# ShifuML/shifu-tensorflow

Hardware: NVIDIA H100
Metric: rows/sec tabular-DNN train (higher is better)
Workload: dtype bf16

## Files before the change

shifu-tensorflow_b200/csrc/capi.cu:

```cuda
#include <math.h>
#include <stdlib.h>
#include <string.h>
#include <algorithm>
#include <memory>
#include <random>
#include "net.cuh"
#include "gemm_dw.cuh"
#include "gemm_pp.cuh"
#include "savedmodel.h"
#include "xchg_p2p.cuh"

using namespace sb;

enum { G_STEP = 0, G_ACC = 1, G_KINDS = 2 };

struct sb_trainer {
  Net net;
  sb_net_desc desc;
  OptHyper hyper;
  float lr = 0.f;
  int rank = 0, world = 1;
  NcclComm comm = nullptr;
  float *grad = nullptr, *s1 = nullptr, *s2 = nullptr, *acc = nullptr;
  int n_acc = 0;
  float grad_out_scale = 1.f;
  long long global_step = 0;
  float* h_scal = nullptr;
  float* d_hscal = nullptr;
  enum { HIST = 8192 };
  float2* h_hist = nullptr;
  float2* d_hist = nullptr;
  float2* hist_slot(long long step) { return d_hist ? d_hist + (step % HIST) : nullptr; }
  float *dsX = nullptr, *dsY = nullptr, *dsW = nullptr;
  __nv_bfloat16* dsXb = nullptr;
  int* dsP = nullptr;
  long long ds_rows = 0;
  std::map<std::pair<int, int>, cudaGraphExec_t> graphs;
  std::map<int, int> kernels_per_step;
  void* xch = nullptr;
  long long xch_n4 = 0;
  long long grad_off = 0, flags_off = 0;
  P2PFlags* flags = nullptr;
  P2PPeers* d_peers = nullptr;
  std::vector<void*> peer_bases;
  bool p2p_ready = false;
  bool peers_share_device = false;
  bool grad_sharded = false;
  bool master_stale = false;
  unsigned int epoch = 0;
  unsigned int* h_err = nullptr;
  unsigned int* d_herr = nullptr;
  unsigned long long xchg_timeout_ns = 300ull * 1000000000ull;
  int xchg_blocks = 0;
  int x_chunks = 1, x_slots = 2;
  int x_chunk_rows = 0;
  int x_begin[SB_XCHG_SLOTS] = {}, x_end[SB_XCHG_SLOTS] = {};
  cudaEvent_t ev_x[SB_XCHG_SLOTS] = {};
  cudaEvent_t ev_c[SB_XCHG_SLOTS] = {};
  bool ll_ready = false;
  long long llg_off = 0, lls_off = 0;
  cudaStream_t side = nullptr;
// ... 1431 lines not shown
  SB_CUDA(cudaMalloc(&dA32, sizeof(float) * M * K));
  SB_CUDA(cudaMalloc(&dB32, sizeof(float) * N * K));
  SB_CUDA(cudaMalloc(&dD, sizeof(float) * M * N));
  SB_CUDA(cudaMalloc(&dA, sizeof(__nv_bfloat16) * a_rows * lda));
  SB_CUDA(cudaMalloc(&dB, sizeof(__nv_bfloat16) * b_rows * ldb));
  SB_CUDA(cudaMemset(dA, 0, sizeof(__nv_bfloat16) * a_rows * lda));
  SB_CUDA(cudaMemset(dB, 0, sizeof(__nv_bfloat16) * b_rows * ldb));
  SB_CUDA(cudaMemset(dD, 0, sizeof(float) * M * N));
  SB_CUDA(cudaMemcpy(dA32, A, sizeof(float) * M * K, cudaMemcpyHostToDevice));
  SB_CUDA(cudaMemcpy(dB32, B, sizeof(float) * N * K, cudaMemcpyHostToDevice));
  cast_bf16_kernel<<<static_cast<unsigned>((static_cast<long long>(M) * K + 255) / 256), 256>>>(dA32, a_rows, a_cols, dA, lda);
  cast_bf16_kernel<<<static_cast<unsigned>((static_cast<long long>(N) * K + 255) / 256), 256>>>(dB32, b_rows, b_cols, dB, ldb);
  GemmPlan pl = plan_gemm(M, N, K, prop.multiProcessorCount, false);
  if (cfg_cg > 0) pl.bn = cfg_bn;
  {
    const int total_kb = (K + 63) / 64;
    int want = split_k < 1 ? 1 : (split_k > total_kb ? total_kb : split_k);
    pl.kb_per_split = (total_kb + want - 1) / want;
    pl.split_k = (total_kb + pl.kb_per_split - 1) / pl.kb_per_split;
    const int work = ((M + 127) / 128) * ((N + pl.bn - 1) / pl.bn) * pl.split_k;
    pl.grid = work < prop.multiProcessorCount ? work : prop.multiProcessorCount;
  }
  TmapSet tms;
  int s = make_tmap_bf16(&tms.a[0], dA, a_rows, a_cols, lda, a_mn ? 64 : 128);
  if (s == SB_OK) s = make_tmap_bf16(&tms.b[0], dB, b_rows, b_cols, ldb, b_mn ? 64 : pl.bn);
  if (s == SB_OK) {
    GemmTcParams p = {};
    p.M = M; p.N = N; p.K = K;
    p.accum = dD; p.ld_acc = N;
    p.acc_vec4 = (N % 4 == 0) ? 1 : 0;
    auto launch = [&]() -> int {
      if (pl.bn == 256) return launch_gemm_dw(pl, tms, p, 0);
      if (!a_mn && !b_mn) return launch_gemm_tc<EPI_F32, false, false>(pl, tms, p, 0);
      if (!a_mn) return launch_gemm_tc<EPI_F32, false, true>(pl, tms, p, 0);
      return launch_gemm_tc<EPI_F32, true, true>(pl, tms, p, 0);
    };
    if (pl.bn == 256) s = set_gemm_dw_attrs();
    else if (!a_mn && !b_mn) s = set_gemm_tc_attrs<EPI_F32, false, false>();
    else if (!a_mn) s = set_gemm_tc_attrs<EPI_F32, false, true>();
    else s = set_gemm_tc_attrs<EPI_F32, true, true>();
    if (s == SB_OK) s = launch();
    if (s == SB_OK && iters > 0) {
      const int ldn = round_up(N, 8);
      float *d_bias = nullptr, *d_colsum = nullptr;
      __nv_bfloat16 *d_out = nullptr, *d_aux = nullptr;
      cudaMalloc(&d_bias, sizeof(float) * N); cudaMemset(d_bias, 0, sizeof(float) * N);
      cudaMalloc(&d_colsum, sizeof(float) * N); cudaMemset(d_colsum, 0, sizeof(float) * N);
      cudaMalloc(&d_out, sizeof(__nv_bfloat16) * static_cast<size_t>(M) * ldn);
      cudaMalloc(&d_aux, sizeof(__nv_bfloat16) * static_cast<size_t>(M) * ldn);
      cudaMemset(d_aux, 0x3f, sizeof(__nv_bfloat16) * static_cast<size_t>(M) * ldn);
      GemmTcParams q = p;
      q.bias = d_bias; q.act = SB_ACT_RELU; q.out = d_out; q.ld_out = ldn; q.aux = d_aux; q.ld_aux = ldn; q.colsum = d_colsum;
      q.acc_vec4 = (N % 4 == 0) ? 1 : 0;
      const PpPlan pp = plan_gemm_pp(M, N, K, prop.multiProcessorCount);
      PpTmaps pt;
      if (!a_mn) {
        if (s == SB_OK) s = make_tmap_bf16(&pt.a, dA, a_rows, a_cols, lda, pp.bm_wg);
        if (s == SB_OK) s = make_tmap_bf16(&pt.b, dB, b_rows, b_cols, ldb, b_mn ? 64 : pp.bn);
        if (s == SB_OK) s = make_tmap_bf16(&pt.o, d_out, M, N, ldn, pp.bm_wg);
        if (s == SB_OK) s = make_tmap_bf16(&pt.x, d_aux, M, N, ldn, pp.bm_wg);
      }
      auto real = [&]() -> int {
        if (!a_mn && !b_mn) return launch_gemm_pp<EPI_DA>(pp, pt, q, 0, false);
        if (!a_mn) return launch_gemm_pp<EPI_FWD>(pp, pt, q, 0, false);
        if (pl.bn == 256) return launch_gemm_dw(pl, tms, q, 0, false);
        return launch_gemm_tc<EPI_DW, true, true>(pl, tms, q, 0, false);
      };
      if (s == SB_OK) s = a_mn ? set_gemm_tc_attrs<EPI_DW, true, true>() : set_gemm_pp_attrs();
      cudaEvent_t e0, e1;
      cudaEventCreate(&e0); cudaEventCreate(&e1);
      for (int i = 0; i < 3 && s == SB_OK; ++i) s = real();
      cudaEventRecord(e0, 0);
      for (int i = 0; i < iters && s == SB_OK; ++i) s = real();
      cudaEventRecord(e1, 0);
      cudaEventSynchronize(e1);
      float ms = 0.f;
      cudaEventElapsedTime(&ms, e0, e1);
      *ms_out = ms / iters;
      cudaEventDestroy(e0); cudaEventDestroy(e1);
      if (getenv("SB_GEMM_TRACE")) {
        unsigned long long* d_tr = nullptr;
        cudaMalloc(&d_tr, 16 * sizeof(unsigned long long));
        cudaMemset(d_tr, 0, 16 * sizeof(unsigned long long));
        q.trace = d_tr;
        cudaDeviceSynchronize();
        cudaEvent_t t0, t1;
        cudaEventCreate(&t0); cudaEventCreate(&t1);
        cudaEventRecord(t0, 0);
        s = real();
        cudaEventRecord(t1, 0);
        cudaEventSynchronize(t1);
        float one = 0.f;
        cudaEventElapsedTime(&one, t0, t1);
        unsigned long long h[16];
        cudaMemcpy(h, d_tr, sizeof(h), cudaMemcpyDeviceToHost);
        if (a_mn)
          fprintf(stderr, "[trace] M=%d N=%d K=%d bn=%d split=%d single-launch %.2f us | ns since entry:", M, N, K, pl.bn, pl.split_k,
                  one * 1e3f);
        else
          fprintf(stderr, "[trace] M=%d N=%d K=%d ping-pong bm_wg=%d bn=%d single-launch %.2f us | ns since entry:", M, N, K, pp.bm_wg,
                  pp.bn, one * 1e3f);
        const char* nm[9] = {"entry", "setup", "deps", "tma0", "land0", "mma_done", "acc_ready", "epi_done", "exit"};
        for (int i = 1; i < 9; ++i) fprintf(stderr, " %s=%lld", nm[i], (long long)(h[i] - h[0]));
        fprintf(stderr, "\n");
        cudaEventDestroy(t0); cudaEventDestroy(t1);
        cudaFree(d_tr);
        q.trace = nullptr;
      }
      cudaFree(d_bias); cudaFree(d_colsum); cudaFree(d_out); cudaFree(d_aux);
    }
  }
  if (s == SB_OK) {
    cudaError_t e = cudaDeviceSynchronize();
    if (e != cudaSuccess) s = set_error(SB_ERR_CUDA, "gemm_tc_kernel failed: %s", cudaGetErrorString(e));
    else if (cudaMemcpy(D, dD, sizeof(float) * M * N, cudaMemcpyDeviceToHost) != cudaSuccess) s = set_error(SB_ERR_CUDA, "D2H failed");
  }
  cudaFree(dA32); cudaFree(dB32); cudaFree(dD); cudaFree(dA); cudaFree(dB);
  return s;
}

extern "C" {
// ... 5 lines not shown
  cudaDeviceProp prop;
  SB_CUDA(cudaGetDeviceProperties(&prop, device));
  SB_CHECK(prop.major == 9 && prop.minor == 0, SB_ERR_CUDA, "device is sm_%d%d, need sm_90", prop.major, prop.minor);
  SB_CUDA(cudaSetDevice(device));
  const int ld = round_up(K, 8);
  const long long a_ps = static_cast<long long>(M) * ld, b_ps = static_cast<long long>(N) * ld;
  float *dA32 = nullptr, *dB32 = nullptr, *dD = nullptr;
  __nv_bfloat16 *dA = nullptr, *dB = nullptr;
  SB_CUDA(cudaMalloc(&dA32, sizeof(float) * M * K));
  SB_CUDA(cudaMalloc(&dB32, sizeof(float) * N * K));
  SB_CUDA(cudaMalloc(&dD, sizeof(float) * M * N));
  SB_CUDA(cudaMalloc(&dA, sizeof(__nv_bfloat16) * a_ps * np));
  SB_CUDA(cudaMalloc(&dB, sizeof(__nv_bfloat16) * b_ps * np));
  SB_CUDA(cudaMemset(dA, 0, sizeof(__nv_bfloat16) * a_ps * np));
  SB_CUDA(cudaMemset(dB, 0, sizeof(__nv_bfloat16) * b_ps * np));
  SB_CUDA(cudaMemset(dD, 0, sizeof(float) * M * N));
  SB_CUDA(cudaMemcpy(dA32, A, sizeof(float) * M * K, cudaMemcpyHostToDevice));
  SB_CUDA(cudaMemcpy(dB32, B, sizeof(float) * N * K, cudaMemcpyHostToDevice));
  cast_bf16_kernel<<<static_cast<unsigned>((static_cast<long long>(M) * K + 255) / 256), 256>>>(dA32, M, K, dA, ld, np, a_ps);
  cast_bf16_kernel<<<static_cast<unsigned>((static_cast<long long>(N) * K + 255) / 256), 256>>>(dB32, N, K, dB, ld, np, b_ps);
  GemmTcParams p = {};
  set_part_pairs(&p, np);
  p.M = M; p.N = N; p.K = K;
  p.accum = dD; p.ld_acc = N;
  const GemmPlan pl = plan_gemm(M, N, round_up(K, 64) * p.n_pairs, prop.multiProcessorCount, false);
  TmapSet tms;
  int s = make_tmaps_bf16(tms.a, dA, a_ps, np, M, K, ld, 128);
  if (s == SB_OK) s = make_tmaps_bf16(tms.b, dB, b_ps, np, N, K, ld, pl.bn);
  if (s == SB_OK) s = set_gemm_tc_attrs<EPI_F32, false, false>();
  if (s == SB_OK) s = launch_gemm_tc<EPI_F32, false, false>(pl, tms, p, 0);
  if (s == SB_OK) {
    cudaError_t e = cudaDeviceSynchronize();
    if (e != cudaSuccess) s = set_error(SB_ERR_CUDA, "gemm_tc_kernel (split) failed: %s", cudaGetErrorString(e));
    else if (cudaMemcpy(D, dD, sizeof(float) * M * N, cudaMemcpyDeviceToHost) != cudaSuccess) s = set_error(SB_ERR_CUDA, "D2H failed");
  }
  cudaFree(dA32); cudaFree(dB32); cudaFree(dD); cudaFree(dA); cudaFree(dB);
  return s;
}

int sb_debug_gemm_bf16_ex(const float* A, const float* B, float* D, int32_t M, int32_t N, int32_t K, int32_t split_k,
                          int32_t a_mn, int32_t b_mn, int device) {
  return sb_debug_gemm_bf16_cfg(A, B, D, M, N, K, split_k, a_mn, b_mn, 0, 0, device);
}
int sb_debug_gemm_bf16(const float* A, const float* B, float* D, int32_t M, int32_t N, int32_t K, int32_t split_k, int device) {
  return sb_debug_gemm_bf16_cfg(A, B, D, M, N, K, split_k, 0, 0, 0, 0, device);
}

int sb_debug_gemm_epilogue(const float* A, const float* W, const float* bias, const float* aux, float* out, float* colsum,
                           int32_t M, int32_t N, int32_t K, int32_t da, int32_t act, int32_t bm_wg, int device,
                           int32_t iters, float* ms_out) {
  SB_CHECK(A && W && out && M > 0 && N > 0 && K > 0 && (da == 0 || da == 1), SB_ERR_INVALID, "bad argument");
  SB_CHECK(da ? aux != nullptr : bias != nullptr, SB_ERR_INVALID, "the forward GEMM needs a bias, the dA GEMM an aux matrix");
  SB_CHECK(act >= SB_ACT_NONE && act <= SB_ACT_LEAKYRELU, SB_ERR_INVALID, "act invalid");
  SB_CHECK(bm_wg == 0 || bm_wg == 64 || bm_wg == 128, SB_ERR_INVALID, "bm_wg must be 0, 64 or 128 (got %d)", bm_wg);
  SB_CHECK(iters >= 0 && (iters == 0 || ms_out != nullptr), SB_ERR_INVALID, "iters / ms_out");
  int n_dev = 0;
  SB_CHECK(cudaGetDeviceCount(&n_dev) == cudaSuccess && n_dev > 0, SB_ERR_CUDA, "no CUDA device available");
  cudaDeviceProp prop;
  SB_CUDA(cudaGetDeviceProperties(&prop, device));
  SB_CHECK(prop.major == 9 && prop.minor == 0, SB_ERR_CUDA, "device is sm_%d%d, need sm_90", prop.major, prop.minor);
  SB_CUDA(cudaSetDevice(device));
  const int w_rows = da ? N : K, w_cols = da ? K : N;
  const int lda = round_up(K, 8), ldw = round_up(w_cols, 8), ldn = round_up(N, 8);
  const size_t mn = static_cast<size_t>(M) * N;
  float *dA32 = nullptr, *dW32 = nullptr, *dX32 = nullptr, *d_bias = nullptr, *d_col = nullptr;
  __nv_bfloat16 *dA = nullptr, *dW = nullptr, *d_out = nullptr, *d_aux = nullptr;
  SB_CUDA(cudaMalloc(&dA32, sizeof(float) * M * K));
  SB_CUDA(cudaMalloc(&dW32, sizeof(float) * N * K));
  SB_CUDA(cudaMalloc(&dX32, sizeof(float) * mn));
  SB_CUDA(cudaMalloc(&d_bias, sizeof(float) * N));
  SB_CUDA(cudaMalloc(&d_col, sizeof(float) * N));
  SB_CUDA(cudaMalloc(&dA, sizeof(__nv_bfloat16) * M * lda));
  SB_CUDA(cudaMalloc(&dW, sizeof(__nv_bfloat16) * w_rows * ldw));
  SB_CUDA(cudaMalloc(&d_out, sizeof(__nv_bfloat16) * M * ldn));
  SB_CUDA(cudaMalloc(&d_aux, sizeof(__nv_bfloat16) * M * ldn));
  SB_CUDA(cudaMemset(dA, 0, sizeof(__nv_bfloat16) * M * lda));
  SB_CUDA(cudaMemset(dW, 0, sizeof(__nv_bfloat16) * w_rows * ldw));
  SB_CUDA(cudaMemset(d_out, 0, sizeof(__nv_bfloat16) * M * ldn));
  SB_CUDA(cudaMemset(d_aux, 0, sizeof(__nv_bfloat16) * M * ldn));
  SB_CUDA(cudaMemset(d_bias, 0, sizeof(float) * N));
  SB_CUDA(cudaMemset(d_col, 0, sizeof(float) * N));
  SB_CUDA(cudaMemcpy(dA32, A, sizeof(float) * M * K, cudaMemcpyHostToDevice));
  SB_CUDA(cudaMemcpy(dW32, W, sizeof(float) * N * K, cudaMemcpyHostToDevice));
  if (bias) SB_CUDA(cudaMemcpy(d_bias, bias, sizeof(float) * N, cudaMemcpyHostToDevice));
  cast_bf16_kernel<<<static_cast<unsigned>((static_cast<long long>(M) * K + 255) / 256), 256>>>(dA32, M, K, dA, lda);
  cast_bf16_kernel<<<static_cast<unsigned>((static_cast<long long>(N) * K + 255) / 256), 256>>>(dW32, w_rows, w_cols, dW, ldw);
  if (aux) {
    SB_CUDA(cudaMemcpy(dX32, aux, sizeof(float) * mn, cudaMemcpyHostToDevice));
    cast_bf16_kernel<<<static_cast<unsigned>((mn + 255) / 256), 256>>>(dX32, M, N, d_aux, ldn);
  }
  const PpPlan pp = plan_gemm_pp(M, N, K, prop.multiProcessorCount, bm_wg);
  PpTmaps pt;
  int s = make_tmap_bf16(&pt.a, dA, M, K, lda, pp.bm_wg);
  if (s == SB_OK) s = make_tmap_bf16(&pt.b, dW, w_rows, w_cols, ldw, da ? pp.bn : 64);
  if (s == SB_OK) s = make_tmap_bf16(&pt.o, d_out, M, N, ldn, pp.bm_wg);
  if (s == SB_OK) s = make_tmap_bf16(&pt.x, d_aux, M, N, ldn, pp.bm_wg);
  GemmTcParams p = {};
  p.M = M; p.N = N; p.K = K;
  p.act = act; p.bias = d_bias; p.colsum = colsum ? d_col : nullptr;
  auto launch = [&]() { return da ? launch_gemm_pp<EPI_DA>(pp, pt, p, 0, false) : launch_gemm_pp<EPI_FWD>(pp, pt, p, 0, false); };
  if (s == SB_OK) s = set_gemm_pp_attrs();
  if (s == SB_OK) s = launch();
  if (s == SB_OK) {
    cudaError_t e = cudaDeviceSynchronize();
    if (e != cudaSuccess) s = set_error(SB_ERR_CUDA, "gemm_pp_kernel failed: %s", cudaGetErrorString(e));
  }
  if (s == SB_OK) {
    std::vector<uint16_t> h(static_cast<size_t>(M) * ldn);
    if (cudaMemcpy(h.data(), d_out, sizeof(uint16_t) * h.size(), cudaMemcpyDeviceToHost) != cudaSuccess) s = set_error(SB_ERR_CUDA, "D2H failed");
    for (int r = 0; r < M && s == SB_OK; ++r)
      for (int c = 0; c < N; ++c) {
        const uint32_t u = static_cast<uint32_t>(h[static_cast<size_t>(r) * ldn + c]) << 16;
        memcpy(out + static_cast<size_t>(r) * N + c, &u, 4);
      }
    if (s == SB_OK && colsum && cudaMemcpy(colsum, d_col, sizeof(float) * N, cudaMemcpyDeviceToHost) != cudaSuccess)
      s = set_error(SB_ERR_CUDA, "D2H failed");
  }
  if (s == SB_OK && iters > 0) {
    cudaEvent_t e0, e1;
    cudaEventCreate(&e0); cudaEventCreate(&e1);
    for (int i = 0; i < 3 && s == SB_OK; ++i) s = launch();
    cudaEventRecord(e0, 0);
    for (int i = 0; i < iters && s == SB_OK; ++i) s = launch();
    cudaEventRecord(e1, 0);
    cudaEventSynchronize(e1);
    float ms = 0.f;
    cudaEventElapsedTime(&ms, e0, e1);
    *ms_out = ms / iters;
    cudaEventDestroy(e0); cudaEventDestroy(e1);
    cudaError_t e = cudaDeviceSynchronize();
    if (s == SB_OK && e != cudaSuccess) s = set_error(SB_ERR_CUDA, "gemm_pp_kernel failed: %s", cudaGetErrorString(e));
  }
  cudaFree(dA32); cudaFree(dW32); cudaFree(dX32); cudaFree(d_bias); cudaFree(d_col);
  cudaFree(dA); cudaFree(dW); cudaFree(d_out); cudaFree(d_aux);
  return s;
}

}
```

shifu-tensorflow_b200/csrc/gemm_pp.cuh:

```cuda
#pragma once
#include "gemm_tc.cuh"

namespace sb {

struct PpTmaps {
  CUtensorMap a;
  CUtensorMap b;
  CUtensorMap o;
  CUtensorMap x;
};

template <int BM_WG, int BN>
struct GemmPpCfg : RingCfg<BM_WG * 64 * 2, BN * 64 * 2, 1024 + 256 + 2 * BN * 4 + 16 * BN * 4 + 2 * BM_WG * BN * 2> {
  static_assert(BM_WG == 64 || BM_WG == 128, "warpgroup tile rows");
  static_assert(BN == 64 || BN == 128, "tile N");
  static_assert(GemmPpCfg::STAGES >= 4, "operand ring");
  static constexpr int X_TILE = BM_WG * 128;
  static constexpr int X_BYTES = X_TILE * (BN / 64);
};

template <int BM_WG, int BN, int EPI, int ACT>
__global__ void __launch_bounds__(GemmPpCfg<BM_WG, BN>::THREADS, 1)
gemm_pp_kernel(const __grid_constant__ PpTmaps tms, const GemmTcParams p) {
  static_assert(EPI == EPI_FWD || EPI == EPI_DA, "forward or dA");
// ... 116 lines not shown
                const uint32_t a = xaddr(64 * mi + r0 + 8 * h, c);
                uint32_t raw;
                asm volatile("ld.shared.b32 %0, [%1];" : "=r"(raw) : "r"(a) : "memory");
                const float x0 = __uint_as_float(raw << 16), x1 = __uint_as_float(raw & 0xFFFF0000u);
                const float v0 = acc[mi][32 * x + 4 * i + 2 * h] * act_grad_from_out(x0, ACT);
                const float v1 = acc[mi][32 * x + 4 * i + 2 * h + 1] * act_grad_from_out(x1, ACT);
                asm volatile("st.shared.b32 [%0], %1;" ::"r"(a), "r"(pack_bf16x2(v0, v1)) : "memory");
                s0 += v0;
                s1 += v1;
              }
            }
            cs[2 * i] = s0;
            cs[2 * i + 1] = s1;
          }
          if (do_cols) {
            colsum_row_groups(cs, lane);
            const uint32_t col = static_cast<uint32_t>(64 * x + c0 + 8 * (lane >> 2));
            asm volatile("st.shared.v2.f32 [%0], {%1, %2};" ::"r"(cb + col * 4u), "f"(cs[0]), "f"(cs[1]) : "memory");
          }
        }
      }
      fence_proxy_async();
      bar_wg();
      if (xthread) {
        for (int x = 0; x < nx; ++x) tma_store_2d(&tms.o, xs + x * Cfg::X_TILE, n0 + x * 64, m0);
        tma_store_commit();
      }
      if (do_cols) {
        const uint32_t cb = col_w + static_cast<uint32_t>((it & 1) * 4 - (warp & 3)) * BN * 4u;
        for (int j = gt; j < BN; j += 128) {
          float v = 0.f;
#pragma unroll
          for (int w = 0; w < 4; ++w) {
            float x;
            asm volatile("ld.shared.f32 %0, [%1];" : "=f"(x) : "r"(cb + (w * BN + j) * 4u) : "memory");
            v += x;
          }
          if (n0 + j < p.N && v != 0.f) red_add_f32(p.colsum + n0 + j, v);
        }
      }
      if (lt == 0 && threadIdx.x == 0) ring_stamp(p, tracing, 7);
    }
    if (xthread) asm volatile("cp.async.bulk.wait_group 0;" ::: "memory");
  }
  ring_exit(p, tracing);
}

struct PpPlan {
  int bm_wg;
  int bn;
  int grid;
};

static inline PpPlan plan_gemm_pp(int M, int N, int K, int num_sms, int bm_wg = 0) {
  PpPlan pl = {};
  pl.bn = N <= 64 ? 64 : 128;
  const int tiles_n = (N + pl.bn - 1) / pl.bn;
  const int tiles128 = ((M + 127) / 128) * tiles_n;
  const bool tall = tiles128 > num_sms || (8 * tiles128 >= 7 * num_sms && (K + 63) / 64 >= 8);
  pl.bm_wg = bm_wg > 0 ? bm_wg : (tall ? 128 : 64);
  const int tiles = ((M + pl.bm_wg - 1) / pl.bm_wg) * tiles_n;
  pl.grid = tiles < num_sms ? tiles : num_sms;
  return pl;
}

template <typename F>
static int with_pp_shape(int bm_wg, int bn, F&& f) {
  using std::integral_constant;
  if (bm_wg == 128 && bn == 128) return f(integral_constant<int, 128>(), integral_constant<int, 128>());
  if (bm_wg == 128 && bn == 64) return f(integral_constant<int, 128>(), integral_constant<int, 64>());
  if (bm_wg == 64 && bn == 128) return f(integral_constant<int, 64>(), integral_constant<int, 128>());
  if (bm_wg == 64 && bn == 64) return f(integral_constant<int, 64>(), integral_constant<int, 64>());
  return set_error(SB_ERR_INVALID, "no gemm_pp instantiation for bm_wg=%d bn=%d", bm_wg, bn);
}

template <int EPI>
static int launch_gemm_pp(const PpPlan& pl, const PpTmaps& tms, const GemmTcParams& p, cudaStream_t st, bool pdl) {
  return with_pp_shape(pl.bm_wg, pl.bn, [&](auto BM_WG, auto BN) {
    return with_act(p.act, [&](auto ACT) {
      using Cfg = GemmPpCfg<BM_WG, BN>;
      return launch_kernel(gemm_pp_kernel<BM_WG, BN, EPI, ACT>, pl.grid, Cfg::THREADS, Cfg::SMEM_BYTES, st, pdl, tms, p);
    });
  });
}

static int set_gemm_pp_attrs() {
  for (int bm_wg : {64, 128})
    for (int bn : {64, 128})
      for (int act = SB_ACT_NONE; act <= SB_ACT_LEAKYRELU; ++act)
        SB_TRY(with_pp_shape(bm_wg, bn, [&](auto BM_WG, auto BN) {
          return with_act(act, [&](auto ACT) {
            const int bytes = GemmPpCfg<BM_WG, BN>::SMEM_BYTES;
            SB_TRY(set_max_smem(gemm_pp_kernel<BM_WG, BN, EPI_FWD, ACT>, bytes));
            return set_max_smem(gemm_pp_kernel<BM_WG, BN, EPI_DA, ACT>, bytes);
          });
        }));
  return SB_OK;
}

}
```

shifu-tensorflow_b200/csrc/net.cu:

```cuda
#include <stdarg.h>
#include <stdlib.h>
#include <string.h>
#include <algorithm>
#include "net.cuh"
#include "gemm_dw.cuh"
#include "gemm_fwd_out.cuh"
#include "gemm_pp.cuh"

namespace sb {

std::string& last_error_ref() {
  thread_local std::string e;
  return e;
}
int set_error(int code, const char* fmt, ...) {
  char buf[1024];
  va_list ap;
  va_start(ap, fmt);
  vsnprintf(buf, sizeof(buf), fmt, ap);
  va_end(ap);
  last_error_ref() = buf;
  return code;
}

PFN_encodeTiled get_encode_tiled() {
  static PFN_encodeTiled fn = nullptr;
  if (!fn) {
    void* p = nullptr;
    cudaDriverEntryPointQueryResult q;
    if (cudaGetDriverEntryPoint("cuTensorMapEncodeTiled", &p, cudaEnableDefault, &q) == cudaSuccess &&
        q == cudaDriverEntryPointSuccess)
      fn = reinterpret_cast<PFN_encodeTiled>(p);
  }
  return fn;
}

int make_tmaps_bf16(CUtensorMap* out3, const void* base, long long part_stride, int np, int rows, int cols, int ld, int box_rows) {
  for (int k = 0; k < (np > 1 ? np : 1); ++k)
    SB_TRY(make_tmap_bf16(out3 + k, static_cast<const __nv_bfloat16*>(base) + k * part_stride, rows, cols, ld, box_rows));
  return SB_OK;
}

void set_part_pairs(GemmTcParams* p, int np) {
  p->np = np > 1 ? np : 1;
  int n = 0;
  for (int sum = p->np - 1; sum >= 0; --sum)
    for (int i = 0; i <= sum; ++i) { p->pair_a[n] = static_cast<unsigned char>(i); p->pair_b[n] = static_cast<unsigned char>(sum - i); ++n; }
  p->n_pairs = n;
}

int make_tmap_bf16(CUtensorMap* out, const void* base, int rows, int cols, int ld, int box_rows) {
  PFN_encodeTiled enc = get_encode_tiled();
  SB_CHECK(enc != nullptr, SB_ERR_CUDA, "cuTensorMapEncodeTiled not available from the driver");
  SB_CHECK(rows > 0 && cols > 0 && (ld % 8) == 0 && (reinterpret_cast<uintptr_t>(base) & 15) == 0, SB_ERR_INVALID,
           "tensor map: bad geometry rows=%d cols=%d ld=%d", rows, cols, ld);
  cuuint64_t gdim[2] = {static_cast<cuuint64_t>(cols), static_cast<cuuint64_t>(rows)};
  cuuint64_t gstr[1] = {static_cast<cuuint64_t>(ld) * 2};
  cuuint32_t box[2] = {64u, static_cast<cuuint32_t>(box_rows)};
  cuuint32_t estr[2] = {1u, 1u};
  CUresult r = enc(out, CU_TENSOR_MAP_DATA_TYPE_BFLOAT16, 2, const_cast<void*>(base), gdim, gstr, box, estr,
// ... 141 lines not shown
  if (bf) {
    Xb_ps = static_cast<long long>(max_batch) * ldF;
    SB_TRY(dalloc(&Xb, static_cast<size_t>(Xb_ps) * nparts));
    A.assign(L, nullptr); dZ.assign(L, nullptr); A_ps.assign(L, 0);
    for (int l = 0; l < L; ++l) {
      Layer& ly = layers[l];
      A_ps[l] = static_cast<long long>(max_batch) * ly.ld_out;
      SB_TRY(dalloc(&A[l], static_cast<size_t>(A_ps[l]) * nparts));
      if (training) SB_TRY(dalloc(&dZ[l], static_cast<size_t>(A_ps[l]) * nparts));
    }
  } else {
    SB_TRY(dalloc(&Xf, static_cast<size_t>(max_batch) * F));
    Af.assign(L, nullptr); dZf.assign(L, nullptr);
    for (int l = 0; l < L; ++l) {
      SB_TRY(dalloc(&Af[l], static_cast<size_t>(max_batch) * layers[l].out));
      if (training) SB_TRY(dalloc(&dZf[l], static_cast<size_t>(max_batch) * layers[l].out));
    }
  }

  std::vector<OptWork> wk;
  auto add_runs = [&](long long o, long long n, const Layer* mat) {
    for (long long s = 0; s < n; s += 1024) {
      OptWork w = {};
      w.off = o + s; w.count = static_cast<int>(n - s < 1024 ? n - s : 1024);
      w.np = 1;
      if (mat) {
        w.out_dim = mat->out; w.mat_off = mat->w_off; w.Wn = mat->Wn; w.ld_out = mat->ld_out;
        w.np = nparts; w.part_stride = Wn_ps[static_cast<size_t>(mat - layers.data())];
      }
      wk.push_back(w);
    }
  };
  work_begin.assign(L + 1, 0); work_end.assign(L + 1, 0);
  for (int l = 0; l <= L; ++l) {
    Layer& ly = layers[l];
    work_begin[l] = static_cast<int>(wk.size());
    if (bf && l < L) {
      add_runs(ly.w_off, static_cast<long long>(ly.in) * ly.out, &ly);
      add_runs(ly.b_off, ly.out, nullptr);
    } else {
      add_runs(ly.w_off, static_cast<long long>(ly.in) * ly.out + ly.out, nullptr);
    }
    work_end[l] = static_cast<int>(wk.size());
  }
  n_work = static_cast<int>(wk.size());
  SB_TRY(dalloc(&work, wk.size()));
  SB_CUDA(cudaMemcpyAsync(work, wk.data(), wk.size() * sizeof(OptWork), cudaMemcpyHostToDevice, stream));
  SB_CUDA(cudaStreamSynchronize(stream));

  if (bf) {
    SB_TRY((set_gemm_tc_attrs<EPI_FWD, false, true>()));
    SB_TRY(set_gemm_fwd_out_attrs());
    SB_TRY(set_gemm_pp_attrs());
    SB_TRY((set_gemm_tc_attrs<EPI_DA, false, false>()));
    SB_TRY((set_gemm_tc_attrs<EPI_DW, true, true>()));
    SB_TRY(set_gemm_dw_attrs());
    const int co = cudaSharedmemCarveoutMaxShared;
    cudaFuncSetAttribute(load_batch_kernel<true>, cudaFuncAttributePreferredSharedMemoryCarveout, co);
    cudaFuncSetAttribute(out_layer_kernel<__nv_bfloat16>, cudaFuncAttributePreferredSharedMemoryCarveout, co);
  }
  return SB_OK;
}

void Net::destroy() {
  if (stream) cudaStreamSynchronize(stream);
  for (void* p : allocs) cudaFree(p);
  allocs.clear();
  if (stream) cudaStreamDestroy(stream);
  stream = nullptr;
}

int Net::set_sparse(int n_dense_, int n_onehot_, int n_cat_) {
  SB_CHECK(n_dense_ >= 1 && n_onehot_ >= 1 && n_cat_ >= 1, SB_ERR_INVALID, "wide+deep needs >= 1 dense, one-hot and categorical column");
  SB_CHECK(n_dense_ + n_onehot_ == F, SB_ERR_INVALID, "n_dense (%d) + n_onehot (%d) must equal n_features (%d): the sparse path evaluates "
           "the SAME first layer", n_dense_, n_onehot_, F);
  SB_CUDA(cudaSetDevice(device));
  n_dense = n_dense_; n_onehot = n_onehot_; n_cat = n_cat_;
  ldD = round_up(n_dense, 8);
  if (!idx) SB_TRY(dalloc(&idx, static_cast<size_t>(max_batch) * n_cat));
  if (!E) SB_TRY(dalloc(&E, static_cast<size_t>(max_batch) * layers[0].ld_out));
  SB_CUDA(cudaStreamSynchronize(stream));
  return SB_OK;
}

int Net::enqueue_embed(int rows, bool scatter, float* grad, cudaStream_t st) {
  const Layer& l0 = layers[0];
  EmbedParams p = {};
  p.rows = rows; p.n_cat = n_cat; p.H = l0.out;
  p.idx = idx;
  p.np = nparts; p.ldW = tc() ? l0.ld_out : l0.out;
  if (tc()) { p.We = l0.Wn + static_cast<size_t>(n_dense) * l0.ld_out; p.We_ps = Wn_ps[0]; }
  else p.We32 = theta + l0.w_off + static_cast<long long>(n_dense) * l0.out;
  p.E = E; p.ldE = l0.ld_out;
  if (scatter) {
    if (tc()) { p.dZ = dZ[0]; p.dZ_ps = A_ps[0]; p.ld_dZ = l0.ld_out; }
    else { p.dZ32 = dZf[0]; p.ld_dZ = l0.out; }
    p.gWe = grad + l0.w_off + static_cast<long long>(n_dense) * l0.out;
    SB_TRY(launch_kernel(embed_scatter_kernel, dim3((rows + 7) / 8), dim3(256), 0, st, false, p));
    mark("embed_scatter");
  } else {
    SB_TRY(launch_kernel(embed_gather_kernel, dim3((rows + 7) / 8), dim3(256), 0, st, false, p));
    mark("embed_gather");
  }
  return SB_OK;
}

// ... 16 lines not shown
    SB_TRY(launch_kernel(load_batch_kernel<true>, dim3(static_cast<unsigned>(blocks)), dim3(256), 0, stream, true,
                         static_cast<const BatchDesc*>(in.desc), rows, Fx, Xb, ldx, static_cast<float*>(nullptr), in.scal, clear,
                         clear_n, nparts, Xb_ps));
  else
    SB_TRY(launch_kernel(load_batch_kernel<false>, dim3(static_cast<unsigned>(blocks)), dim3(256), 0, stream, true,
                         static_cast<const BatchDesc*>(in.desc), rows, Fx, static_cast<__nv_bfloat16*>(nullptr), ldx, Xf, in.scal,
                         clear, clear_n, 1, 0ll));
  mark("load_batch");
  if (in.sparse) SB_TRY(enqueue_embed(rows, false, nullptr, stream));
  return SB_OK;
}

int Net::enqueue_hidden_forward(const StepIn& in, int rows, float* grad, bool* fused_out, float4* clear, long long clear_n4) {
  if (fused_out) *fused_out = false;
  for (int l = 0; l < L; ++l) {
    Layer& ly = layers[l];
    const bool sp0 = (l == 0) && in.sparse;
    const int k_in = sp0 ? n_dense : ly.in;
    const int ld_k = sp0 ? ldD : ly.ld_in;
    if (tc()) {
      TmapSet tm;
      const bool res0 = (l == 0) && in.resident;
      const __nv_bfloat16* src = (l == 0) ? (res0 ? resident_Xb : Xb) : A[l - 1];
      const long long src_ps = (l == 0) ? (res0 ? resident_ps : Xb_ps) : A_ps[l - 1];
      const int src_rows = res0 ? static_cast<int>(resident_rows) : rows;
      SB_TRY(make_tmaps_bf16(tm.b, ly.Wn, Wn_ps[l], nparts, k_in, ly.out, ly.ld_out, 64));
      GemmTcParams p = {};
      set_part_pairs(&p, nparts);
      p.M = rows; p.N = ly.out; p.K = k_in;
      if (sp0) { p.addend = E; p.ld_add = ly.ld_out; }
      p.bias = theta + ly.b_off; p.act = ly.act;
      p.out = A[l]; p.ld_out = ly.ld_out; p.out_ps = A_ps[l];
      p.a_rows = res0 ? in.desc : nullptr;
      if (l == L - 1 && grad != nullptr && training && ly.out <= FWD_OUT_MAX_N && p.addend == nullptr) {
        FwdOutTmaps ft;
        SB_TRY(make_tmaps_bf16(ft.a, src, src_ps, nparts, src_rows, k_in, ld_k, 64));
        for (int i = 0; i < 3; ++i) ft.b[i] = tm.b[i];
        SB_TRY(make_tmaps_bf16(ft.o, dZ[l], A_ps[l], nparts, rows, ly.out, ly.ld_out, 64));
        const int tiles = (rows + 63) / 64;
        const int grid = tiles < num_sms ? tiles : num_sms;
        Layer& ol = layers[L];
        p.wo = theta + ol.w_off; p.bo = theta + ol.b_off;
        p.desc = in.desc; p.scal = in.scal; p.loss = loss;
        p.g_wo = grad + ol.w_off; p.g_bo = grad + ol.b_off; p.g_bL = grad + ly.b_off;
        p.trace = next_trace("fwd_out", l, rows, ly.out, k_in);
        SB_TRY(launch_gemm_fwd_out(grid, ft, p, stream, true));
        if (fused_out) *fused_out = true;
        mark("gemm_fwd_out");
        continue;
      }
      if (l == 0) { p.zero_buf = clear; p.zero_n4 = clear_n4; }
      p.trace = next_trace("fwd", l, rows, ly.out, k_in);
      if (nparts == 1 && p.addend == nullptr) {
        const PpPlan pp = plan_gemm_pp(rows, ly.out, k_in, num_sms);
        PpTmaps pt;
        SB_TRY(make_tmap_bf16(&pt.a, src, src_rows, k_in, ld_k, pp.bm_wg));
        pt.b = tm.b[0];
        SB_TRY(make_tmap_bf16(&pt.o, A[l], rows, ly.out, ly.ld_out, pp.bm_wg));
        SB_TRY(launch_gemm_pp<EPI_FWD>(pp, pt, p, stream, true));
      } else {
        const GemmPlan pl = plan_gemm(rows, ly.out, round_up(k_in, 64) * pairs_of(nparts), num_sms, false);
        SB_TRY(make_tmaps_bf16(tm.a, src, src_ps, nparts, src_rows, k_in, ld_k, 128));
        SB_TRY((launch_gemm_tc<EPI_FWD, false, true>(pl, tm, p, stream, true)));
      }
    } else {
      GemmF32Params p = {};
      p.M = rows; p.N = ly.out; p.K = k_in;
      p.A = (l == 0) ? Xf : Af[l - 1]; p.sAm = k_in; p.sAk = 1;
      if (sp0) { p.addend = E; p.ld_add = ly.ld_out; }
      p.B = theta + ly.w_off; p.sBk = ly.out; p.sBn = 1;
      p.bias = theta + ly.b_off; p.act = ly.act;
      p.out = Af[l]; p.ld_out = ly.out;
      SB_TRY(launch_gemm_f32<EPI_FWD>(p, 1, stream));
    }
    mark("gemm_fwd");
  }
  return SB_OK;
}

int Net::enqueue_out(const StepIn& in, int rows, bool do_loss, bool do_bwd, float* yhat_dst, float* grad) {
  Layer& hl = layers[L - 1];
  Layer& ol = layers[L];
  OutLayerParams p = {};
  p.rows = rows; p.H = hl.out;
  p.wo = theta + ol.w_off; p.bo = theta + ol.b_off;
  p.desc = in.desc; p.scal = in.scal; p.loss = loss; p.act = hl.act;
  p.do_bwd = do_bwd ? 1 : 0; p.do_loss = do_loss ? 1 : 0;
  p.yhat = yhat_dst;
  p.trace = next_trace("out_layer");
  if (do_bwd) {
    p.g_wo = grad + ol.w_off; p.g_bo = grad + ol.b_off; p.g_bL = grad + hl.b_off;
  }
  const int grid = (rows + 31) / 32;
  if (tc()) {
    p.A = A[L - 1]; p.ldA = hl.ld_out;
    p.np = nparts; p.a_ps = A_ps[L - 1]; p.dz_ps = A_ps[L - 1];
    if (do_bwd) { p.dZ = dZ[L - 1]; p.ld_dZ = hl.ld_out; }
    if (hl.out <= 1024) {
      int rpb = (rows + 2 * num_sms - 1) / (2 * num_sms);
      rpb = ((rpb + 7) / 8) * 8;
      if (rpb < 8) rpb = 8;
      const dim3 g((rows + rpb - 1) / rpb);
      if (hl.out <= 256) SB_TRY(launch_kernel(out_layer_rows_kernel<1>, g, dim3(256), 0, stream, true, p, rpb));
      else if (hl.out <= 512) SB_TRY(launch_kernel(out_layer_rows_kernel<2>, g, dim3(256), 0, stream, true, p, rpb));
      else SB_TRY(launch_kernel(out_layer_rows_kernel<4>, g, dim3(256), 0, stream, true, p, rpb));
    } else {
      SB_TRY(launch_kernel(out_layer_kernel<__nv_bfloat16>, dim3(grid), dim3(256), 0, stream, true, p));
    }
  } else {
    p.A = Af[L - 1]; p.ldA = hl.out;
    if (do_bwd) { p.dZ = dZf[L - 1]; p.ld_dZ = hl.out; }
    SB_TRY(launch_kernel(out_layer_kernel<float>, dim3(grid), dim3(256), 0, stream, true, p));
// ... 19 lines not shown
    int split = (2 * num_sms) / (tiles > 0 ? tiles : 1);
    const int cap = (rows + 63) / 64;
    if (split > cap) split = cap;
    SB_TRY(launch_gemm_f32<EPI_DW>(p, split, st));
    mark("gemm_dw");
    return SB_OK;
  }
  const bool res0 = (l == 0) && in.resident;
  const int ld_k = sp0 ? ldD : ly.ld_in;
  const __nv_bfloat16* ap = (l == 0) ? (res0 ? resident_Xb : Xb) : A[l - 1];
  const long long ap_ps = (l == 0) ? (res0 ? resident_ps : Xb_ps) : A_ps[l - 1];
  const GemmPlan pl = plan_gemm(r1 - r0, ly.out, round_up(rows, 64) * pairs_of(nparts), sms, true);
  TmapSet tm;
  SB_TRY(make_tmaps_bf16(tm.a, ap + r0, ap_ps, nparts, res0 ? static_cast<int>(resident_rows) : rows, r1 - r0, ld_k, 64));
  SB_TRY(make_tmaps_bf16(tm.b, dZ[l], A_ps[l], nparts, rows, ly.out, ly.ld_out, 64));
  GemmTcParams p = {};
  set_part_pairs(&p, nparts);
  p.M = r1 - r0; p.N = ly.out; p.K = rows;
  p.a_rows = res0 ? in.desc : nullptr;
  p.accum = grad + ly.w_off + static_cast<long long>(r0) * ly.out; p.ld_acc = ly.out;
  p.acc_vec4 = (ly.out % 4 == 0 && ly.w_off % 4 == 0) ? 1 : 0;
  p.trace = next_trace("dW", l, r1 - r0, ly.out, rows, chunk);
  if (pl.bn == 256) SB_TRY(launch_gemm_dw(pl, tm, p, st, pdl));
  else SB_TRY((launch_gemm_tc<EPI_DW, true, true>(pl, tm, p, st, pdl)));
  mark("gemm_dw");
  return SB_OK;
}

int Net::enqueue_da(int l, int rows, float* grad) {
  Layer& ly = layers[l];
  Layer& pl = layers[l - 1];
  if (!tc()) {
    GemmF32Params p = {};
    p.M = rows; p.N = ly.in; p.K = ly.out;
    p.A = dZf[l]; p.sAm = ly.out; p.sAk = 1;
    p.B = theta + ly.w_off; p.sBk = 1; p.sBn = ly.out;
    p.act = pl.act;
    p.aux = Af[l - 1]; p.ld_aux = pl.out;
    p.out = dZf[l - 1]; p.ld_out = pl.out;
    p.colsum = grad + pl.b_off;
    SB_TRY(launch_gemm_f32<EPI_DA>(p, 1, stream));
    mark("gemm_da");
    return SB_OK;
  }
  GemmTcParams p = {};
  set_part_pairs(&p, nparts);
  p.M = rows; p.N = ly.in; p.K = ly.out;
  p.act = pl.act;
  p.aux = A[l - 1]; p.ld_aux = pl.ld_out; p.aux_ps = A_ps[l - 1];
  p.out = dZ[l - 1]; p.ld_out = pl.ld_out; p.out_ps = A_ps[l - 1];
  p.colsum = grad + pl.b_off;
  p.trace = next_trace("dA", l, rows, ly.in, ly.out);
  if (nparts == 1) {
    const PpPlan pp = plan_gemm_pp(rows, ly.in, ly.out, num_sms);
    PpTmaps pt;
    SB_TRY(make_tmap_bf16(&pt.a, dZ[l], rows, ly.out, ly.ld_out, pp.bm_wg));
    SB_TRY(make_tmap_bf16(&pt.b, ly.Wn, ly.in, ly.out, ly.ld_out, pp.bn));
    SB_TRY(make_tmap_bf16(&pt.o, dZ[l - 1], rows, ly.in, pl.ld_out, pp.bm_wg));
    SB_TRY(make_tmap_bf16(&pt.x, A[l - 1], rows, ly.in, pl.ld_out, pp.bm_wg));
    SB_TRY(launch_gemm_pp<EPI_DA>(pp, pt, p, stream, true));
  } else {
    const GemmPlan gp = plan_gemm(rows, ly.in, round_up(ly.out, 64) * pairs_of(nparts), num_sms, false);
    TmapSet tm;
    SB_TRY(make_tmaps_bf16(tm.a, dZ[l], A_ps[l], nparts, rows, ly.out, ly.ld_out, 128));
    SB_TRY(make_tmaps_bf16(tm.b, ly.Wn, Wn_ps[l], nparts, ly.in, ly.out, ly.ld_out, gp.bn));
    SB_TRY((launch_gemm_tc<EPI_DA, false, false>(gp, tm, p, stream, true)));
  }
  mark("gemm_da");
  return SB_OK;
}
}
```

Measured before the change: 35.62 million.

## Add 128x256-tile forward GEMM kernel for wide layers with enough K depth

Adds a new warp-specialized forward GEMM kernel that uses 128x256 output tiles, with bias plus activation epilogue and TMA stores. The planner picks it for forward layers when N exceeds 128, K spans at least 16 blocks, and the wider tiles at least halve the number of waves. The goal is better operand reuse per loaded A tile and fewer tile passes on deep, wide layers. In exchange it needs more shared memory and registers per CTA, and the tile grid gets coarser, which can hurt load balance.

Result: faster. 37.73 million, median of 6 (+5.9%).

```diff
diff --git a/shifu-tensorflow_b200/csrc/capi.cu b/shifu-tensorflow_b200/csrc/capi.cu
--- a/shifu-tensorflow_b200/csrc/capi.cu
+++ b/shifu-tensorflow_b200/csrc/capi.cu
@@ -7,6 +7,7 @@
 #include "net.cuh"
 #include "gemm_dw.cuh"
 #include "gemm_pp.cuh"
+#include "gemm_wide.cuh"
 #include "savedmodel.h"
 #include "xchg_p2p.cuh"
 
@@ -1544,7 +1545,7 @@
       GemmTcParams q = p;
       q.bias = d_bias; q.act = SB_ACT_RELU; q.out = d_out; q.ld_out = ldn; q.aux = d_aux; q.ld_aux = ldn; q.colsum = d_colsum;
       q.acc_vec4 = (N % 4 == 0) ? 1 : 0;
-      const PpPlan pp = plan_gemm_pp(M, N, K, prop.multiProcessorCount);
+      const PpPlan pp = plan_gemm_pp(M, N, K, prop.multiProcessorCount, !a_mn && b_mn);
       PpTmaps pt;
       if (!a_mn) {
         if (s == SB_OK) s = make_tmap_bf16(&pt.a, dA, a_rows, a_cols, lda, pp.bm_wg);
@@ -1554,11 +1555,12 @@
       }
       auto real = [&]() -> int {
         if (!a_mn && !b_mn) return launch_gemm_pp<EPI_DA>(pp, pt, q, 0, false);
-        if (!a_mn) return launch_gemm_pp<EPI_FWD>(pp, pt, q, 0, false);
+        if (!a_mn) return pp.bn == 256 ? launch_gemm_wide(pp, pt, q, 0, false) : launch_gemm_pp<EPI_FWD>(pp, pt, q, 0, false);
         if (pl.bn == 256) return launch_gemm_dw(pl, tms, q, 0, false);
         return launch_gemm_tc<EPI_DW, true, true>(pl, tms, q, 0, false);
       };
       if (s == SB_OK) s = a_mn ? set_gemm_tc_attrs<EPI_DW, true, true>() : set_gemm_pp_attrs();
+      if (s == SB_OK && pp.bn == 256) s = set_gemm_wide_attrs();
       cudaEvent_t e0, e1;
       cudaEventCreate(&e0); cudaEventCreate(&e1);
       for (int i = 0; i < 3 && s == SB_OK; ++i) s = real();
@@ -1670,7 +1672,9 @@
   SB_CHECK(A && W && out && M > 0 && N > 0 && K > 0 && (da == 0 || da == 1), SB_ERR_INVALID, "bad argument");
   SB_CHECK(da ? aux != nullptr : bias != nullptr, SB_ERR_INVALID, "the forward GEMM needs a bias, the dA GEMM an aux matrix");
   SB_CHECK(act >= SB_ACT_NONE && act <= SB_ACT_LEAKYRELU, SB_ERR_INVALID, "act invalid");
-  SB_CHECK(bm_wg == 0 || bm_wg == 64 || bm_wg == 128, SB_ERR_INVALID, "bm_wg must be 0, 64 or 128 (got %d)", bm_wg);
+  SB_CHECK(bm_wg == 0 || bm_wg == 64 || bm_wg == 128 || bm_wg == PP_TILE_WIDE, SB_ERR_INVALID,
+           "bm_wg must be 0, 64, 128 or %d (got %d)", PP_TILE_WIDE, bm_wg);
+  SB_CHECK(!(da && bm_wg == PP_TILE_WIDE), SB_ERR_INVALID, "the %d-wide tile is for the forward GEMM only", PP_TILE_WIDE);
   SB_CHECK(iters >= 0 && (iters == 0 || ms_out != nullptr), SB_ERR_INVALID, "iters / ms_out");
   int n_dev = 0;
   SB_CHECK(cudaGetDeviceCount(&n_dev) == cudaSuccess && n_dev > 0, SB_ERR_CUDA, "no CUDA device available");
@@ -1707,7 +1711,7 @@
     SB_CUDA(cudaMemcpy(dX32, aux, sizeof(float) * mn, cudaMemcpyHostToDevice));
     cast_bf16_kernel<<<static_cast<unsigned>((mn + 255) / 256), 256>>>(dX32, M, N, d_aux, ldn);
   }
-  const PpPlan pp = plan_gemm_pp(M, N, K, prop.multiProcessorCount, bm_wg);
+  const PpPlan pp = plan_gemm_pp(M, N, K, prop.multiProcessorCount, da == 0, bm_wg);
   PpTmaps pt;
   int s = make_tmap_bf16(&pt.a, dA, M, K, lda, pp.bm_wg);
   if (s == SB_OK) s = make_tmap_bf16(&pt.b, dW, w_rows, w_cols, ldw, da ? pp.bn : 64);
@@ -1716,12 +1720,15 @@
   GemmTcParams p = {};
   p.M = M; p.N = N; p.K = K;
   p.act = act; p.bias = d_bias; p.colsum = colsum ? d_col : nullptr;
-  auto launch = [&]() { return da ? launch_gemm_pp<EPI_DA>(pp, pt, p, 0, false) : launch_gemm_pp<EPI_FWD>(pp, pt, p, 0, false); };
-  if (s == SB_OK) s = set_gemm_pp_attrs();
+  auto launch = [&]() {
+    if (da) return launch_gemm_pp<EPI_DA>(pp, pt, p, 0, false);
+    return pp.bn == 256 ? launch_gemm_wide(pp, pt, p, 0, false) : launch_gemm_pp<EPI_FWD>(pp, pt, p, 0, false);
+  };
+  if (s == SB_OK) s = pp.bn == 256 ? set_gemm_wide_attrs() : set_gemm_pp_attrs();
   if (s == SB_OK) s = launch();
   if (s == SB_OK) {
     cudaError_t e = cudaDeviceSynchronize();
-    if (e != cudaSuccess) s = set_error(SB_ERR_CUDA, "gemm_pp_kernel failed: %s", cudaGetErrorString(e));
+    if (e != cudaSuccess) s = set_error(SB_ERR_CUDA, "%s failed: %s", pp.bn == 256 ? "gemm_wide_kernel" : "gemm_pp_kernel", cudaGetErrorString(e));
   }
   if (s == SB_OK) {
     std::vector<uint16_t> h(static_cast<size_t>(M) * ldn);
diff --git a/shifu-tensorflow_b200/csrc/gemm_pp.cuh b/shifu-tensorflow_b200/csrc/gemm_pp.cuh
--- a/shifu-tensorflow_b200/csrc/gemm_pp.cuh
+++ b/shifu-tensorflow_b200/csrc/gemm_pp.cuh
@@ -192,13 +192,25 @@
   int grid;
 };
 
-static inline PpPlan plan_gemm_pp(int M, int N, int K, int num_sms, int bm_wg = 0) {
+constexpr int PP_TILE_WIDE = 256;
+
+static inline PpPlan plan_gemm_pp(int M, int N, int K, int num_sms, bool fwd, int tile = 0) {
   PpPlan pl = {};
+  const int tiles_m = (M + 127) / 128, kb = (K + 63) / 64;
+  const int wide_tiles = tiles_m * ((N + 255) / 256), narrow_tiles = tiles_m * ((N + 127) / 128);
+  const bool wide = fwd && N > 128 && 8 * wide_tiles >= 7 * num_sms && kb >= 16 &&
+                    2 * ((wide_tiles + num_sms - 1) / num_sms) <= (narrow_tiles + num_sms - 1) / num_sms;
+  if (tile == PP_TILE_WIDE || (tile == 0 && wide)) {
+    pl.bm_wg = 128;
+    pl.bn = 256;
+    pl.grid = wide_tiles < num_sms ? wide_tiles : num_sms;
+    return pl;
+  }
   pl.bn = N <= 64 ? 64 : 128;
   const int tiles_n = (N + pl.bn - 1) / pl.bn;
-  const int tiles128 = ((M + 127) / 128) * tiles_n;
-  const bool tall = tiles128 > num_sms || (8 * tiles128 >= 7 * num_sms && (K + 63) / 64 >= 8);
-  pl.bm_wg = bm_wg > 0 ? bm_wg : (tall ? 128 : 64);
+  const int tiles128 = tiles_m * tiles_n;
+  const bool tall = tiles128 > num_sms || (8 * tiles128 >= 7 * num_sms && kb >= 8);
+  pl.bm_wg = tile > 0 ? tile : (tall ? 128 : 64);
   const int tiles = ((M + pl.bm_wg - 1) / pl.bm_wg) * tiles_n;
   pl.grid = tiles < num_sms ? tiles : num_sms;
   return pl;
diff --git a/shifu-tensorflow_b200/csrc/gemm_wide.cuh b/shifu-tensorflow_b200/csrc/gemm_wide.cuh
--- /dev/null
+++ b/shifu-tensorflow_b200/csrc/gemm_wide.cuh
@@ -0,0 +1,115 @@
+#pragma once
+#include "gemm_pp.cuh"
+
+namespace sb {
+
+struct GemmWideCfg : RingCfg<128 * 64 * 2, 256 * 64 * 2, 1024 + 256 + 256 * 4 + 128 * 256 * 2> {
+  static constexpr int BM = 128, BN = 256;
+  static constexpr int X_TILE = BM * 128;
+};
+static_assert(GemmWideCfg::STAGES >= 3, "operand ring");
+
+template <int ACT>
+__global__ void __launch_bounds__(GemmWideCfg::THREADS, 1)
+gemm_wide_kernel(const __grid_constant__ PpTmaps tms, const GemmTcParams p) {
+  using Cfg = GemmWideCfg;
+  constexpr int BM = Cfg::BM, BN = Cfg::BN, BK = Cfg::BK;
+
+  extern __shared__ uint8_t smem_raw[];
+  const Ring<Cfg> ring(smem_raw, Cfg::BN * Cfg::BM * 2);
+  const uint32_t xs = ring.end();
+  const uint32_t bias_s = ring.bars + 256u;
+
+  const int warp = threadIdx.x >> 5;
+  const int lane = threadIdx.x & 31;
+  const bool tracing = ring_enter(ring, 2, 0, &tms.a, &tms.b, p);
+
+  const int tiles_m = (p.M + BM - 1) / BM;
+  const int tiles_n = (p.N + BN - 1) / BN;
+  const int n_tiles = tiles_m * tiles_n;
+  const int kb_n = (p.K + BK - 1) / BK;
+
+  if (warp >= Cfg::PRODUCER_WARP) {
+    asm volatile("setmaxnreg.dec.sync.aligned.u32 %0;" ::"n"(Cfg::PRODUCER_REGS));
+    if (warp == Cfg::PRODUCER_WARP && lane == 0) {
+      RingPos<Cfg::STAGES> pos;
+      const int a_row0 = (p.a_rows != nullptr) ? p.a_rows->row0 : 0;
+      for (int t = blockIdx.x; t < n_tiles; t += gridDim.x) {
+        const int m0 = (t / tiles_n) * BM, n0 = (t % tiles_n) * BN;
+        for (int kb = 0; kb < kb_n; ++kb) {
+          ring_issue(ring, pos, [&](uint32_t fb, uint32_t sa, uint32_t sb) {
+            tma_load_2d(sa, &tms.a, fb, kb * BK, m0 + a_row0);
+#pragma unroll
+            for (int j = 0; j < BN / 64; ++j) tma_load_2d(sb + j * 8192, &tms.b, fb, n0 + j * 64, kb * BK);
+          });
+          if (kb == 0 && t == static_cast<int>(blockIdx.x)) ring_stamp(p, tracing, 3);
+        }
+      }
+    }
+    ring_producer_tail<Cfg>(p);
+  } else {
+    asm volatile("setmaxnreg.inc.sync.aligned.u32 %0;" ::"n"(Cfg::CONSUMER_REGS));
+    const int g = warp >> 2;
+    const int ct = static_cast<int>(threadIdx.x);
+    auto bar_consumers = [&]() { asm volatile("bar.sync 2, 256;" ::: "memory"); };
+    const int r0 = 64 * g + (warp & 3) * 16 + (lane >> 2);
+    const int c0 = 2 * (lane & 3);
+    auto xaddr = [&](int r, int c) {
+      return xs + static_cast<uint32_t>((c >> 6) * Cfg::X_TILE + r * 128 + ((((c & 63) >> 3) ^ (r & 7)) << 4) + (c & 7) * 2);
+    };
+
+    float acc_mi[1][BN / 2];
+    float (&acc)[BN / 2] = acc_mi[0];
+    RingPos<Cfg::STAGES> pos;
+    for (int t = blockIdx.x; t < n_tiles; t += gridDim.x) {
+      const bool first = t == static_cast<int>(blockIdx.x);
+      const int m0 = (t / tiles_n) * BM, n0 = (t % tiles_n) * BN;
+      const int nx = min(BN / 64, (p.N - n0 + 63) / 64);
+      const float bv = (n0 + ct < p.N) ? __ldg(p.bias + n0 + ct) : 0.f;
+
+      ring_mma<BN, false, true>(ring, pos, kb_n, acc_mi, static_cast<uint32_t>(g) * 8192u, 0u, (ct & 127) == 0, first, p,
+                                tracing);
+
+      asm volatile("st.shared.f32 [%0], %1;" ::"r"(bias_s + ct * 4u), "f"(bv) : "memory");
+      if (ct == 0) tma_store_wait_read<0>();
+      bar_consumers();
+#pragma unroll
+      for (int i = 0; i < BN / 8; ++i) {
+        const int c = c0 + 8 * i;
+        float2 b;
+        asm volatile("ld.shared.v2.f32 {%0, %1}, [%2];" : "=f"(b.x), "=f"(b.y) : "r"(bias_s + c * 4u) : "memory");
+#pragma unroll
+        for (int h = 0; h < 2; ++h) {
+          const float v0 = act_apply(acc[4 * i + 2 * h] + b.x, ACT);
+          const float v1 = act_apply(acc[4 * i + 2 * h + 1] + b.y, ACT);
+          asm volatile("st.shared.b32 [%0], %1;" ::"r"(xaddr(r0 + 8 * h, c)), "r"(pack_bf16x2(v0, v1)) : "memory");
+        }
+      }
+      fence_proxy_async();
+      bar_consumers();
+      if (ct == 0) {
+        for (int x = 0; x < nx; ++x) tma_store_2d(&tms.o, xs + x * Cfg::X_TILE, n0 + x * 64, m0);
+        tma_store_commit();
+      }
+      if (first && ct == 0) ring_stamp(p, tracing, 7);
+    }
+    if (ct == 0) asm volatile("cp.async.bulk.wait_group 0;" ::: "memory");
+  }
+  ring_exit(p, tracing);
+}
+
+static int launch_gemm_wide(const PpPlan& pl, const PpTmaps& tms, const GemmTcParams& p, cudaStream_t st, bool pdl) {
+  if (pl.bm_wg != GemmWideCfg::BM || pl.bn != GemmWideCfg::BN)
+    return set_error(SB_ERR_INVALID, "gemm_wide has 128 x 256 tiles only (bm_wg=%d bn=%d)", pl.bm_wg, pl.bn);
+  return with_act(p.act, [&](auto ACT) {
+    return launch_kernel(gemm_wide_kernel<ACT>, pl.grid, GemmWideCfg::THREADS, GemmWideCfg::SMEM_BYTES, st, pdl, tms, p);
+  });
+}
+
+static int set_gemm_wide_attrs() {
+  for (int act = SB_ACT_NONE; act <= SB_ACT_LEAKYRELU; ++act)
+    SB_TRY(with_act(act, [&](auto ACT) { return set_max_smem(gemm_wide_kernel<ACT>, GemmWideCfg::SMEM_BYTES); }));
+  return SB_OK;
+}
+
+}
diff --git a/shifu-tensorflow_b200/csrc/net.cu b/shifu-tensorflow_b200/csrc/net.cu
--- a/shifu-tensorflow_b200/csrc/net.cu
+++ b/shifu-tensorflow_b200/csrc/net.cu
@@ -6,6 +6,7 @@
 #include "gemm_dw.cuh"
 #include "gemm_fwd_out.cuh"
 #include "gemm_pp.cuh"
+#include "gemm_wide.cuh"
 
 namespace sb {
 
@@ -253,6 +254,7 @@
     SB_TRY((set_gemm_tc_attrs<EPI_FWD, false, true>()));
     SB_TRY(set_gemm_fwd_out_attrs());
     SB_TRY(set_gemm_pp_attrs());
+    SB_TRY(set_gemm_wide_attrs());
     SB_TRY((set_gemm_tc_attrs<EPI_DA, false, false>()));
     SB_TRY((set_gemm_tc_attrs<EPI_DW, true, true>()));
     SB_TRY(set_gemm_dw_attrs());
@@ -375,12 +377,13 @@
       if (l == 0) { p.zero_buf = clear; p.zero_n4 = clear_n4; }
       p.trace = next_trace("fwd", l, rows, ly.out, k_in);
       if (nparts == 1 && p.addend == nullptr) {
-        const PpPlan pp = plan_gemm_pp(rows, ly.out, k_in, num_sms);
+        const PpPlan pp = plan_gemm_pp(rows, ly.out, k_in, num_sms, true);
         PpTmaps pt;
         SB_TRY(make_tmap_bf16(&pt.a, src, src_rows, k_in, ld_k, pp.bm_wg));
         pt.b = tm.b[0];
         SB_TRY(make_tmap_bf16(&pt.o, A[l], rows, ly.out, ly.ld_out, pp.bm_wg));
-        SB_TRY(launch_gemm_pp<EPI_FWD>(pp, pt, p, stream, true));
+        if (pp.bn == 256) SB_TRY(launch_gemm_wide(pp, pt, p, stream, true));
+        else SB_TRY(launch_gemm_pp<EPI_FWD>(pp, pt, p, stream, true));
       } else {
         const GemmPlan pl = plan_gemm(rows, ly.out, round_up(k_in, 64) * pairs_of(nparts), num_sms, false);
         SB_TRY(make_tmaps_bf16(tm.a, src, src_ps, nparts, src_rows, k_in, ld_k, 128));
@@ -506,7 +509,7 @@
   p.colsum = grad + pl.b_off;
   p.trace = next_trace("dA", l, rows, ly.in, ly.out);
   if (nparts == 1) {
-    const PpPlan pp = plan_gemm_pp(rows, ly.in, ly.out, num_sms);
+    const PpPlan pp = plan_gemm_pp(rows, ly.in, ly.out, num_sms, false);
     PpTmaps pt;
     SB_TRY(make_tmap_bf16(&pt.a, dZ[l], rows, ly.out, ly.ld_out, pp.bm_wg));
     SB_TRY(make_tmap_bf16(&pt.b, ly.Wn, ly.in, ly.out, ly.ld_out, pp.bn));
```
